# PKU-VCL-Geometry/GeoSplatting

Hardware: AMD Instinct MI355X
Metric: fwd+bwd views/sec at 2M Gaussians, 800x800 (higher is better)
Workload: dtype f32

## Files before the change

### geosplatting_amd/csrc/gs_cube.h

```cpp
#pragma once
#include "gs_common.h"

struct FaceMap { int a, b, c; float sx, sy; };
__device__ __forceinline__ FaceMap face_map(int s)
{
    const int axis = s >> 1;
    FaceMap m;
    m.a = axis == 0 ? 2 : 0;
    m.b = axis == 1 ? 2 : 1;
    m.c = axis;
    m.sx = (s == 0 || s == 5) ? -1.0f : 1.0f;
    m.sy = s == 2 ? 1.0f : -1.0f;
    return m;
}

__device__ __forceinline__ int select_face(const float* d)
{
    const float ax = fabsf(d[0]), ay = fabsf(d[1]), az = fabsf(d[2]);
    int f; float c;
    if (az > fmaxf(ax, ay)) { f = 4; c = d[2]; }
    else if (ay > ax)       { f = 2; c = d[1]; }
    else                    { f = 0; c = d[0]; }
    return f + (c < 0.0f ? 1 : 0);
}
// ... 12 lines not shown

__device__ __forceinline__ float comp3(const float* d, int i) { return i == 0 ? d[0] : (i == 1 ? d[1] : d[2]); }

__device__ __attribute__((noinline)) int resolve_texel_reproject(int s, int ix, int iy, int R)
{
    const float xn = 2.0f * (((float)ix + 0.5f) / (float)R) - 1.0f;
    const float yn = 2.0f * (((float)iy + 0.5f) / (float)R) - 1.0f;
    float p[3];
    face_point(s, xn, yn, p);
    const int s2 = select_face(p);
    const FaceMap m = face_map(s2);
    const float inv = 1.0f / fabsf(comp3(p, m.c));
    const float x2 = m.sx * comp3(p, m.a) * inv, y2 = m.sy * comp3(p, m.b) * inv;
    const float tx = (x2 + 1.0f) * 0.5f * (float)R - 0.5f, ty = (y2 + 1.0f) * 0.5f * (float)R - 0.5f;
    int jx = (int)floorf(tx + 0.5f), jy = (int)floorf(ty + 0.5f);
    jx = min(max(jx, 0), R - 1); jy = min(max(jy, 0), R - 1);
    return (s2 * R + jy) * R + jx;
}

#define GS_CUBE_EDGE_TABLE_MAX_R 4096
__device__ __forceinline__ int resolve_texel(int s, int ix, int iy, int R)
{
    const bool ox = (ix < 0 || ix >= R), oy = (iy < 0 || iy >= R);
    if (!ox && !oy) return (s * R + iy) * R + ix;
    if (ox && oy) return -1;
    const int e = ox ? (ix < 0 ? 0 : 1) : (iy < 0 ? 2 : 3);
    const int t = ox ? iy : ix;
    const unsigned w = s == 0 ? 0x97aa2ccu : s == 1 ? 0xc70a24du : s == 2 ? 0x2874c11u : s == 3 ? 0x7ad1839u : s == 4 ? 0x26ca049u : 0x766a0c8u;
    const unsigned c = (w >> (7 * e)) & 127u;
    const int s2 = (int)(c & 7u), kx = (int)((c >> 3) & 3u), ky = (int)((c >> 5) & 3u);
    const int jx = kx == 0 ? 0 : (kx == 1 ? R - 1 : (kx == 2 ? t : R - 1 - t));
    const int jy = ky == 0 ? 0 : (ky == 1 ? R - 1 : (ky == 2 ? t : R - 1 - t));
    return (s2 * R + jy) * R + jx;
}

struct CubeFp {
    bool valid;
    int idx[4];
    float w[4];
    float fx, fy;
    int face;
    float inv_c, xn, yn;
};

__device__ void cube_footprint(const float* d, int R, CubeFp& fp)
{
    const int s = select_face(d);
    const FaceMap m = face_map(s);
    const float ac = fabsf(comp3(d, m.c));
    fp.valid = (ac > 0.0f) && isfinite(ac);
    fp.face = s;
    if (!fp.valid) { fp.idx[0] = fp.idx[1] = fp.idx[2] = fp.idx[3] = 0; return; }
    const float inv = 1.0f / ac;
    const float xn = m.sx * comp3(d, m.a) * inv, yn = m.sy * comp3(d, m.b) * inv;
    fp.inv_c = inv; fp.xn = xn; fp.yn = yn;
    const float tx = (xn + 1.0f) * 0.5f * (float)R - 0.5f, ty = (yn + 1.0f) * 0.5f * (float)R - 0.5f;
    const int ix0 = (int)floorf(tx), iy0 = (int)floorf(ty);
    const float fx = tx - (float)ix0, fy = ty - (float)iy0;
    fp.fx = fx; fp.fy = fy;
    if (ix0 >= 0 && iy0 >= 0 && ix0 + 1 < R && iy0 + 1 < R) {
        const int b = (s * R + iy0) * R + ix0;
        fp.idx[0] = b; fp.idx[1] = b + 1; fp.idx[2] = b + R; fp.idx[3] = b + R + 1;
    } else {
        fp.idx[0] = resolve_texel(s, ix0, iy0, R);
        fp.idx[1] = resolve_texel(s, ix0 + 1, iy0, R);
        fp.idx[2] = resolve_texel(s, ix0, iy0 + 1, R);
        fp.idx[3] = resolve_texel(s, ix0 + 1, iy0 + 1, R);
    }
    float w[4] = { (1.0f - fx) * (1.0f - fy), fx * (1.0f - fy), (1.0f - fx) * fy, fx * fy };
    int miss = -1;
#pragma unroll
    for (int i = 0; i < 4; ++i) if (fp.idx[i] < 0) miss = i;
#pragma unroll
    for (int i = 0; i < 4; ++i) fp.w[i] = w[i];
    if (miss >= 0) {
        float wm = 0.0f;
#pragma unroll
        for (int i = 0; i < 4; ++i) if (i == miss) wm = w[i] / 3.0f;
#pragma unroll
        for (int i = 0; i < 4; ++i) fp.w[i] = (i == miss) ? 0.0f : w[i] + wm;
    }
}

template <bool WITH_GRAD>
__device__ void cube_fetch(const float* __restrict__ tex, int R, const float* d, float* out, float* dd, CubeFp& fp)
{
    cube_footprint(d, R, fp);
    const bool valid = fp.valid;
    bool ok[4]; int safe[4];
#pragma unroll
    for (int i = 0; i < 4; ++i) { ok[i] = valid && fp.idx[i] >= 0; safe[i] = ok[i] ? fp.idx[i] : 0; }
    float t[4][3];
#pragma unroll
    for (int i = 0; i < 4; ++i) {
        const float* p = tex + (size_t)safe[i] * 3;
        t[i][0] = p[0]; t[i][1] = p[1]; t[i][2] = p[2];
    }
    bool has_miss = false;
#pragma unroll
    for (int i = 0; i < 4; ++i) {
        if (!ok[i]) { t[i][0] = t[i][1] = t[i][2] = 0.0f; }
        has_miss = has_miss || (valid && fp.idx[i] < 0);
    }
    if (has_miss) {
#pragma unroll
        for (int c = 0; c < 3; ++c) {
            const float s = (t[0][c] + t[1][c] + t[2][c] + t[3][c]) / 3.0f;
#pragma unroll
            for (int i = 0; i < 4; ++i) if (fp.idx[i] < 0) t[i][c] = s;
        }
    }
    if (!valid) {
        out[0] = out[1] = out[2] = 0.0f;
        if (WITH_GRAD) { for (int i = 0; i < 9; ++i) dd[i] = 0.0f; }
        return;
    }
    const FaceMap m = face_map(fp.face);
    const float sgn_c = comp3(d, m.c) < 0.0f ? -1.0f : 1.0f;
#pragma unroll
    for (int c = 0; c < 3; ++c) {
        const float top = t[0][c] + fp.fx * (t[1][c] - t[0][c]);
        const float bot = t[2][c] + fp.fx * (t[3][c] - t[2][c]);
        out[c] = top + fp.fy * (bot - top);
        if (WITH_GRAD) {
            const float dtx = (t[1][c] - t[0][c]) + fp.fy * ((t[3][c] - t[2][c]) - (t[1][c] - t[0][c]));
            const float dty = bot - top;
            const float gx = dtx * 0.5f * (float)R, gy = dty * 0.5f * (float)R;
            float g[3] = { 0.0f, 0.0f, 0.0f };
            const float va = gx * m.sx * fp.inv_c, vb = gy * m.sy * fp.inv_c;
            const float vc = -(gx * fp.xn + gy * fp.yn) * fp.inv_c * sgn_c;
#pragma unroll
            for (int k = 0; k < 3; ++k) g[k] = (k == m.a ? va : 0.0f) + (k == m.b ? vb : 0.0f) + (k == m.c ? vc : 0.0f);
            dd[c * 3 + 0] = g[0]; dd[c * 3 + 1] = g[1]; dd[c * 3 + 2] = g[2];
        }
    }
}

template <bool XCD_LOCAL>
__device__ __forceinline__ void gs_add_scoped(float* p, float v)
{
    if (XCD_LOCAL) gs_atomic_add_xcd(p, v); else gs_atomic_add(p, v);
}

template <bool XCD_LOCAL>
__device__ __forceinline__ void wave_commit6_lds(float* stage, float* pa, float* pb, const float (&v)[6])
{
    const int lane = (int)(threadIdx.x & 63);
    unsigned long long* sp = reinterpret_cast<unsigned long long*>(stage);
    float* sv = stage + 256;
    __builtin_amdgcn_wave_barrier();
    sp[lane] = (unsigned long long)pa; sp[64 + lane] = (unsigned long long)pb;
#pragma unroll
    for (int c = 0; c < 6; ++c) sv[c * 64 + lane] = v[c];
    __builtin_amdgcn_fence(__ATOMIC_RELEASE, "wavefront");
    __builtin_amdgcn_wave_barrier();
    __builtin_amdgcn_fence(__ATOMIC_ACQUIRE, "wavefront");
#pragma unroll
    for (int k = 0; k < 6; ++k) {
        const int q = 64 * k + lane;
        const int src = q / 6, ch = q - 6 * src;
        const bool second = ch >= 3;
        float* base = (float*)sp[(second ? 64 : 0) + src];
        const float val = sv[ch * 64 + src];
        if (base != nullptr) gs_add_scoped<XCD_LOCAL>(base + (second ? ch - 3 : ch), val);
    }
}
// ... 86 lines not shown
```

### geosplatting_amd/csrc/gs_shade.hip

```cpp
#include "gs_common.h"
#include <stdlib.h>
#include <math.h>

#pragma clang fp contract(off)
#include "gs_shade_dev.h"

__global__ void __launch_bounds__(256)
shade_fwd_kernel(int N, const float* __restrict__ means, const float* __restrict__ normals,
                 const float* __restrict__ kd, const float* __restrict__ ks, const float* __restrict__ cam_pos,
                 float min_roughness, float max_metallic, int mode, EnvDev env, float* __restrict__ colors)
{
    const int n = blockIdx.x * blockDim.x + threadIdx.x;
    if (n >= N) return;
    const float mean[3] = { means[3 * (size_t)n], means[3 * (size_t)n + 1], means[3 * (size_t)n + 2] };
    const float nrm[3] = { normals[3 * (size_t)n], normals[3 * (size_t)n + 1], normals[3 * (size_t)n + 2] };
    const float kdn[3] = { kd[3 * (size_t)n], kd[3 * (size_t)n + 1], kd[3 * (size_t)n + 2] };
    const float2 ks2 = *reinterpret_cast<const float2*>(ks + 2 * (size_t)n);
    const float ksn[2] = { ks2.x, ks2.y };
    const float cp[3] = { cam_pos[0], cam_pos[1], cam_pos[2] };
    ShadeTmp t;
    float color[3];
    shade_one<false>(mean, nrm, kdn, ksn, cp, min_roughness, max_metallic, mode, env, color, t);
    colors[3 * (size_t)n] = color[0]; colors[3 * (size_t)n + 1] = color[1]; colors[3 * (size_t)n + 2] = color[2];
}

template <bool PRIV>
__global__ void __launch_bounds__(GS_SHADE_BWD_BLOCK)
shade_bwd_kernel(int N, const float* __restrict__ means, const float* __restrict__ normals,
                 const float* __restrict__ kd, const float* __restrict__ ks, const float* __restrict__ cam_pos,
                 float min_roughness, float max_metallic, int mode, EnvDev env, const float* __restrict__ v_colors,
                 float* __restrict__ v_means, float* __restrict__ v_normals, float* __restrict__ v_kd,
                 float* __restrict__ v_ks, EnvGradDev eg, int accumulate)
{
    extern __shared__ __attribute__((aligned(16))) float s_grad[];
    for (int i = threadIdx.x; i < eg.lds_floats; i += blockDim.x) s_grad[i] = 0.0f;
    __syncthreads();
    float* const priv = PRIV ? eg.priv + (long long)gs_xcc_id() * eg.priv_stride : nullptr;
    float* const stage = s_grad + eg.stage_off + (threadIdx.x >> 6) * 640;
    const float cp[3] = { cam_pos[0], cam_pos[1], cam_pos[2] };
    const int n_iter = (N + (int)(gridDim.x * blockDim.x) - 1) / (int)(gridDim.x * blockDim.x);
    for (int it = 0; it < n_iter; ++it) {
        const int n = it * (int)(gridDim.x * blockDim.x) + blockIdx.x * blockDim.x + threadIdx.x;
        bool scatter = false;
        ShadeTmp t;
        float v_ls[3] = { 0, 0, 0 }, v_ld[3] = { 0, 0, 0 };
        if (n < N) {
            const float mean[3] = { means[3 * (size_t)n], means[3 * (size_t)n + 1], means[3 * (size_t)n + 2] };
            const float normal[3] = { normals[3 * (size_t)n], normals[3 * (size_t)n + 1], normals[3 * (size_t)n + 2] };
            const float kdn[3] = { kd[3 * (size_t)n], kd[3 * (size_t)n + 1], kd[3 * (size_t)n + 2] };
            const float2 ks2 = *reinterpret_cast<const float2*>(ks + 2 * (size_t)n);
            const float ksn[2] = { ks2.x, ks2.y };
            const float g[3] = { v_colors[3 * (size_t)n], v_colors[3 * (size_t)n + 1], v_colors[3 * (size_t)n + 2] };
            if (g[0] == 0.0f && g[1] == 0.0f && g[2] == 0.0f) {
#pragma unroll
                for (int k = 0; k < 3; ++k) {
                    if (!accumulate) { v_means[3 * (size_t)n + k] = 0.0f; v_normals[3 * (size_t)n + k] = 0.0f; v_kd[3 * (size_t)n + k] = 0.0f; }
                }
                if (!accumulate) *reinterpret_cast<float2*>(v_ks + 2 * (size_t)n) = make_float2(0.0f, 0.0f);
            } else {
                float color[3], o_mean[3], v_n[3], o_kd[3], o_ks[2];
                shade_one<true>(mean, normal, kdn, ksn, cp, min_roughness, max_metallic, mode, env, color, t);
                shade_one_bwd(t, normal, kdn, g, mode, min_roughness, max_metallic, v_ls, v_ld, o_kd, v_n, o_ks, o_mean);
                scatter = true;
                if (accumulate) {
#pragma unroll
                    for (int k = 0; k < 3; ++k) {
                        v_means[3 * (size_t)n + k] += o_mean[k];
                        v_normals[3 * (size_t)n + k] += v_n[k];
                        v_kd[3 * (size_t)n + k] += o_kd[k];
                    }
                    float2 o = *reinterpret_cast<float2*>(v_ks + 2 * (size_t)n);
                    o.x += o_ks[0]; o.y += o_ks[1];
                    *reinterpret_cast<float2*>(v_ks + 2 * (size_t)n) = o;
                } else {
#pragma unroll
                    for (int k = 0; k < 3; ++k) {
                        v_means[3 * (size_t)n + k] = o_mean[k];
                        v_normals[3 * (size_t)n + k] = v_n[k];
                        v_kd[3 * (size_t)n + k] = o_kd[k];
                    }
                    *reinterpret_cast<float2*>(v_ks + 2 * (size_t)n) = make_float2(o_ks[0], o_ks[1]);
                }
            }
        }
        if (mode != GS_MODE_DIFFUSE) {
            const int l0 = scatter ? t.ls.l0 : 0, l1 = scatter ? t.ls.l1 : -1;
            const float w0 = (l1 < 0) ? 1.0f : 1.0f - t.ls.f;
            const bool lds0 = scatter && eg.lds_level[l0] >= 0;
            if (lds0) cube_scatter_lds(s_grad + eg.lds_level[l0], t.ls.fp0, v_ls, w0);
            cube_scatter_wave<PRIV>(scatter && !lds0 ? (PRIV ? priv + eg.priv_level[l0] : eg.levels[l0]) : nullptr, t.ls.fp0,
                                    v_ls, w0, scatter && !lds0, stage);
            const bool has1 = scatter && l1 >= 0;
            const bool lds1 = has1 && eg.lds_level[has1 ? l1 : 0] >= 0;
            if (lds1) cube_scatter_lds(s_grad + eg.lds_level[l1], t.ls.fp1, v_ls, t.ls.f);
            cube_scatter_wave<PRIV>(has1 && !lds1 ? (PRIV ? priv + eg.priv_level[has1 ? l1 : 0] : eg.levels[l1]) : nullptr,
                                    t.ls.fp1, v_ls, t.ls.f, has1 && !lds1, stage);
        } else {
            const bool ldsb = scatter && eg.lds_base >= 0;
            if (ldsb) cube_scatter_lds(s_grad + eg.lds_base, t.ld_fp, v_ld, 1.0f);
            cube_scatter_wave<PRIV>(scatter && !ldsb ? (PRIV ? priv + eg.priv_base : eg.base) : nullptr, t.ld_fp, v_ld, 1.0f,
                                    scatter && !ldsb, stage);
        }
    }
    __syncthreads();
    env_lds_flush(s_grad, eg, env);
// ... 131 lines not shown
        const float gx = g.x * tone_grad(mode, r * e), gy = g.y * tone_grad(mode, gch * e), gz = g.z * tone_grad(mode, b * e);
        v_render[3 * p] = gx * e; v_render[3 * p + 1] = gy * e; v_render[3 * p + 2] = gz * e;
        v_alphas[p] = mode == GS_TONE_NONE ? g.w * e : g.w;
        ve += gx * r + gy * gch + gz * b + (mode == GS_TONE_NONE ? g.w * a : 0.0f);
    }
    ve = gs_wave_sum(ve);
    __shared__ float s[4];
    if ((threadIdx.x & 63) == 0) s[threadIdx.x >> 6] = ve;
    __syncthreads();
    if (threadIdx.x == 0) gs_atomic_add(v_exposure, s[0] + s[1] + s[2] + s[3]);
}

extern "C" int gs_tonemap_fwd3(int64_t P, int mode, const float* render, const float* alphas, const float* exposure, float* out,
                               void* stream)
{
    GS_CHECK_ARG(P >= 0 && mode >= 0 && mode <= 2, "bad P or mode");
    if (P == 0) return GS_OK;
    const int blocks = (int)((P + 255) / 256 < 2048 ? (P + 255) / 256 : 2048);
    hipLaunchKernelGGL(tonemap_fwd3_kernel, dim3(blocks), dim3(256), 0, (hipStream_t)stream, P, mode, render, alphas, exposure, (float4*)out);
    GS_CHECK_LAUNCH();
    return GS_OK;
}

extern "C" int gs_tonemap_bwd3(int64_t P, int mode, const float* render, const float* alphas, const float* exposure,
                               const float* v_out, float* v_render, float* v_alphas, float* v_exposure, int accumulate, void* stream)
{
    GS_CHECK_ARG(P >= 0 && mode >= 0 && mode <= 2, "bad P or mode");
    hipStream_t s = (hipStream_t)stream;
    if (!accumulate) GS_CHECK_HIP(gs_zero_async(v_exposure, sizeof(float), s));
    if (P == 0) return GS_OK;
    const int blocks = (int)((P + 255) / 256 < 1024 ? (P + 255) / 256 : 1024);
    hipLaunchKernelGGL(tonemap_bwd3_kernel, dim3(blocks), dim3(256), 0, s, P, mode, render, alphas, exposure, (const float4*)v_out,
                       v_render, v_alphas, v_exposure);
    GS_CHECK_LAUNCH();
    return GS_OK;
}

extern "C" int gs_tonemap_fwd(int64_t P, int mode, const float* rgba, const float* exposure, float* out, void* stream)
{
    GS_CHECK_ARG(P >= 0 && mode >= 0 && mode <= 2, "bad P or mode");
    if (P == 0) return GS_OK;
    const int blocks = (int)((P + 255) / 256 < 2048 ? (P + 255) / 256 : 2048);
    hipLaunchKernelGGL(tonemap_fwd_kernel, dim3(blocks), dim3(256), 0, (hipStream_t)stream, P, mode,
                       (const float4*)rgba, exposure, (float4*)out);
    GS_CHECK_LAUNCH();
    return GS_OK;
}

extern "C" int gs_tonemap_bwd(int64_t P, int mode, const float* rgba, const float* exposure, const float* v_out,
                              float* v_rgba, float* v_exposure, int accumulate, void* stream)
{
    GS_CHECK_ARG(P >= 0 && mode >= 0 && mode <= 2, "bad P or mode");
    hipStream_t s = (hipStream_t)stream;
    if (!accumulate) GS_CHECK_HIP(gs_zero_async(v_exposure, sizeof(float), s));
    if (P == 0) return GS_OK;
    const int blocks = (int)((P + 255) / 256 < 1024 ? (P + 255) / 256 : 1024);
    hipLaunchKernelGGL(tonemap_bwd_kernel, dim3(blocks), dim3(256), 0, s, P, mode, (const float4*)rgba, exposure,
                       (const float4*)v_out, (float4*)v_rgba, v_exposure);
    GS_CHECK_LAUNCH();
    return GS_OK;
}

__global__ void __launch_bounds__(256) selftest_cube_edges_kernel(int R, unsigned long long* mismatches)
{
    const long long total = 24ll * R;
    unsigned long long bad = 0;
    for (long long i = (long long)blockIdx.x * blockDim.x + threadIdx.x; i < total; i += (long long)gridDim.x * blockDim.x) {
        const int t = (int)(i % R), e = (int)((i / R) & 3), s = (int)(i / (4ll * R));
        const int ix = e == 0 ? -1 : (e == 1 ? R : t), iy = e == 2 ? -1 : (e == 3 ? R : t);
        bad += resolve_texel(s, ix, iy, R) != resolve_texel_reproject(s, ix, iy, R);
    }
    if (bad) atomicAdd(mismatches, bad);
}

extern "C" int gs_selftest_cube_edges(int R, uint64_t* mismatches_dev, void* stream)
{
    GS_CHECK_ARG(mismatches_dev != nullptr && R >= 1 && R <= GS_CUBE_EDGE_TABLE_MAX_R, "bad size");
    hipStream_t s = (hipStream_t)stream;
    GS_CHECK_HIP(gs_zero_async(mismatches_dev, sizeof(uint64_t), s));
    hipLaunchKernelGGL(selftest_cube_edges_kernel, dim3(gs_cdiv(24 * R, 256)), dim3(256), 0, s, R, (unsigned long long*)mismatches_dev);
    GS_CHECK_LAUNCH();
    return GS_OK;
}
```

### geosplatting_amd/csrc/gs_shade_dev.h

```cpp
#pragma once
#include "gs_common.h"
#include <stdlib.h>
#include <math.h>
#include "gs_cube.h"

struct EnvDev {
    const float* lut; int lut_res;
    const float* base; int base_res;
    int L;
    const float* levels[GS_MAX_LEVELS];
    int res[GS_MAX_LEVELS];
    float min_r, max_r;
};
struct EnvGradDev {
    float* base;
    float* levels[GS_MAX_LEVELS];
    int lds_base;
    int lds_level[GS_MAX_LEVELS];
    int lds_floats;
    int stage_off;
    float* priv;
    long long priv_stride;
    long long priv_level[GS_MAX_LEVELS];
    long long priv_base;
// ... 53 lines not shown
    m.l0 = last ? L - 1 : lf;
    m.l1 = last ? -1 : lf + 1;
    m.f = last ? 0.0f : lam - (float)m.l0;
    m.clamped = last || (bias < 0.0f || bias > (float)(L - 1));
    return m;
}

struct MipSample {
    float out[3], dd[9], dmip[3];
    CubeFp fp0, fp1;
    float f;
    int l0, l1;
};

template <bool WITH_GRAD>
__device__ void cube_mip_fetch(const EnvDev& env, const float* d, float bias, MipSample& s)
{
    const int L = env.L;
    const float lam = fminf(fmaxf(bias, 0.0f), (float)(L - 1));
    const int lf = (int)floorf(lam);
    const bool last = lf >= L - 1;
    const int l0 = last ? L - 1 : lf;
    const int l1 = last ? L - 1 : lf + 1;
    const float f = last ? 0.0f : lam - (float)l0;
    float c0[3], c1[3], dd0[9], dd1[9];
    cube_fetch<WITH_GRAD>(env.levels[l0], env.res[l0], d, c0, dd0, s.fp0);
    cube_fetch<WITH_GRAD>(env.levels[l1], env.res[l1], d, c1, dd1, s.fp1);
    s.l0 = l0; s.l1 = last ? -1 : l1; s.f = f;
    const bool clamped = last || (bias < 0.0f || bias > (float)(L - 1));
#pragma unroll
    for (int c = 0; c < 3; ++c) {
        s.out[c] = c0[c] + f * (c1[c] - c0[c]);
        s.dmip[c] = clamped ? 0.0f : (c1[c] - c0[c]);
        if (WITH_GRAD) {
#pragma unroll
            for (int k = 0; k < 3; ++k) s.dd[c * 3 + k] = dd0[c * 3 + k] + f * (dd1[c * 3 + k] - dd0[c * 3 + k]);
        }
    }
}

struct ShadeTmp {
    float rough, metal, spec[3], diff[3];
    float wo[3], len; bool wo_const;
    float d, ndv, fg[2], dfg_du[2], dfg_dv[2];
    float refl[3], mip, dmip_dr;
    MipSample ls;
    float ld[3], ld_dd[9]; CubeFp ld_fp;
    float refl_c[3];
};

template <bool WITH_GRAD>
__device__ void shade_one(const float* mean, const float* normal, const float* kd, const float* ks, const float* cam_pos,
                          float min_roughness, float max_metallic, int mode, const EnvDev& env, float* color, ShadeTmp& t)
{
    t.rough = ks[0] * (1.0f - min_roughness) + min_roughness;
    t.metal = ks[1] * max_metallic;
#pragma unroll
    for (int c = 0; c < 3; ++c) {
        t.spec[c] = (1.0f - t.metal) * 0.04f + kd[c] * t.metal;
        t.diff[c] = kd[c] * (1.0f - t.metal);
    }
    const float v[3] = { cam_pos[0] - mean[0], cam_pos[1] - mean[1], cam_pos[2] - mean[2] };
    const float len = sqrtf(v[0] * v[0] + v[1] * v[1] + v[2] * v[2]);
    t.len = len;
    if (len < 1e-6f) { t.wo[0] = 0.0f; t.wo[1] = 0.0f; t.wo[2] = 1.0f; t.wo_const = true; }
    else { const float l = fmaxf(len, 1e-6f); t.wo[0] = v[0] / l; t.wo[1] = v[1] / l; t.wo[2] = v[2] / l; t.wo_const = false; }
    t.d = normal[0] * t.wo[0] + normal[1] * t.wo[1] + normal[2] * t.wo[2];
    t.ndv = fmaxf(t.d, 1e-6f);
    tex2d_linear_clamp2(env.lut, env.lut_res, env.lut_res, t.ndv, t.rough, t.fg, t.dfg_du, t.dfg_dv);
#pragma unroll
    for (int k = 0; k < 3; ++k) t.refl[k] = 2.0f * t.d * normal[k] - t.wo[k];
    t.mip = mip_from_roughness(t.rough, env.min_r, env.max_r, env.L, t.dmip_dr);
    if (mode != GS_MODE_DIFFUSE) cube_mip_fetch<WITH_GRAD>(env, t.refl, t.mip, t.ls);
    else { t.ls.out[0] = t.ls.out[1] = t.ls.out[2] = 0.0f; }
    if (mode == GS_MODE_DIFFUSE) cube_fetch<WITH_GRAD>(env.base, env.base_res, normal, t.ld, t.ld_dd, t.ld_fp);
    else { t.ld[0] = t.ld[1] = t.ld[2] = 0.0f; }
#pragma unroll
    for (int c = 0; c < 3; ++c) {
        t.refl_c[c] = t.spec[c] * t.fg[0] + t.fg[1];
        if (mode == GS_MODE_PBR)          color[c] = t.diff[c] + t.ls.out[c] * t.refl_c[c];
        else if (mode == GS_MODE_DIFFUSE) color[c] = t.ld[c] * t.diff[c];
        else                              color[c] = t.ls.out[c] * t.refl_c[c];
    }
}

__device__ __forceinline__ void shade_one_bwd(const ShadeTmp& t, const float* normal, const float* kd, const float* g, int mode,
                                              float min_roughness, float max_metallic, float* v_ls, float* v_ld, float* o_kd, float* v_n,
                                              float* v_ks, float* o_mean)
{
    float v_diff[3] = { 0, 0, 0 }, v_rf[3] = { 0, 0, 0 };
#pragma unroll
    for (int c = 0; c < 3; ++c) {
        if (mode == GS_MODE_PBR)          { v_diff[c] = g[c]; v_ls[c] = g[c] * t.refl_c[c]; v_rf[c] = g[c] * t.ls.out[c]; }
        else if (mode == GS_MODE_DIFFUSE) { v_ld[c] = g[c] * t.diff[c]; v_diff[c] = g[c] * t.ld[c]; }
        else                              { v_ls[c] = g[c] * t.refl_c[c]; v_rf[c] = g[c] * t.ls.out[c]; }
    }
    float v_A = 0.0f, v_B = 0.0f, v_metal = 0.0f;
#pragma unroll
    for (int c = 0; c < 3; ++c) {
        const float v_spec = v_rf[c] * t.fg[0];
        v_A += v_rf[c] * t.spec[c];
        v_B += v_rf[c];
        o_kd[c] = v_spec * t.metal + v_diff[c] * (1.0f - t.metal);
        v_metal += v_spec * (kd[c] - 0.04f) - v_diff[c] * kd[c];
    }
    const float v_ndv = v_A * t.dfg_du[0] + v_B * t.dfg_du[1];
    float v_rough = v_A * t.dfg_dv[0] + v_B * t.dfg_dv[1];
    float v_mip = 0.0f, v_refl[3] = { 0, 0, 0 };
    v_n[0] = v_n[1] = v_n[2] = 0.0f;
    if (mode != GS_MODE_DIFFUSE) {
#pragma unroll
        for (int c = 0; c < 3; ++c) {
            v_mip += v_ls[c] * t.ls.dmip[c];
#pragma unroll
            for (int k = 0; k < 3; ++k) v_refl[k] += v_ls[c] * t.ls.dd[c * 3 + k];
        }
    } else {
#pragma unroll
        for (int c = 0; c < 3; ++c)
#pragma unroll
            for (int k = 0; k < 3; ++k) v_n[k] += v_ld[c] * t.ld_dd[c * 3 + k];
    }
    v_rough += v_mip * t.dmip_dr;
    float v_d = 2.0f * (v_refl[0] * normal[0] + v_refl[1] * normal[1] + v_refl[2] * normal[2]);
    float v_wo[3];
#pragma unroll
    for (int k = 0; k < 3; ++k) { v_n[k] += 2.0f * t.d * v_refl[k]; v_wo[k] = -v_refl[k]; }
    if (t.d >= 1e-6f) v_d += v_ndv;
#pragma unroll
    for (int k = 0; k < 3; ++k) { v_n[k] += v_d * t.wo[k]; v_wo[k] += v_d * normal[k]; }
    o_mean[0] = o_mean[1] = o_mean[2] = 0.0f;
    if (!t.wo_const) {
        const float dot = t.wo[0] * v_wo[0] + t.wo[1] * v_wo[1] + t.wo[2] * v_wo[2];
        const float l = fmaxf(t.len, 1e-6f);
#pragma unroll
        for (int k = 0; k < 3; ++k) o_mean[k] = -((v_wo[k] - t.wo[k] * dot) / l);
    }
    v_ks[0] = v_rough * (1.0f - min_roughness); v_ks[1] = v_metal * max_metallic;
}

__device__ __forceinline__ void cube_fetch_vjp(const float* __restrict__ tex, int R, const float* d, const float* v, float* out,
                                               float& s, float* v_d, CubeFp& fp)
{
    cube_footprint(d, R, fp);
    const bool valid = fp.valid;
    bool ok[4]; int safe[4];
#pragma unroll
    for (int i = 0; i < 4; ++i) { ok[i] = valid && fp.idx[i] >= 0; safe[i] = ok[i] ? fp.idx[i] : 0; }
    float t[4][3];
#pragma unroll
    for (int i = 0; i < 4; ++i) {
        const float* p = tex + (size_t)safe[i] * 3;
        t[i][0] = p[0]; t[i][1] = p[1]; t[i][2] = p[2];
    }
    bool has_miss = false;
#pragma unroll
    for (int i = 0; i < 4; ++i) {
        if (!ok[i]) { t[i][0] = t[i][1] = t[i][2] = 0.0f; }
        has_miss = has_miss || (valid && fp.idx[i] < 0);
    }
    if (has_miss) {
#pragma unroll
        for (int c = 0; c < 3; ++c) {
            const float m = (t[0][c] + t[1][c] + t[2][c] + t[3][c]) / 3.0f;
#pragma unroll
            for (int i = 0; i < 4; ++i) if (fp.idx[i] < 0) t[i][c] = m;
// ... 261 lines not shown
```

### include/geosplat_hip.h

```cpp
#ifndef GEOSPLAT_HIP_H
#define GEOSPLAT_HIP_H

#include <stddef.h>
#include <stdint.h>

#ifdef __cplusplus
extern "C" {
#endif

#define GS_OK            0
#define GS_EINVAL       -1
#define GS_ENOSPC       -2
#define GS_ELAUNCH      -3

#define GS_MAX_LEVELS   16
#define GS_MAX_CHANNELS 32

#define GS_MODE_PBR      0
#define GS_MODE_DIFFUSE  1
#define GS_MODE_SPECULAR 2
#define GS_TONE_NONE     0
#define GS_TONE_NAIVE    1
#define GS_TONE_ACES     2

// ... 52 lines not shown
size_t gs_raster_ws_bytes(int64_t n_isects, int V, int W, int H, int tile_size);

int gs_raster_fwd(int W, int H, int tile_size, int D, int V, const float* means2d, const float* conics,
                  const float* opacities, const float* colors, const float* background,
                  int64_t n_isects, const int32_t* offsets, const int32_t* flatten_ids,
                  float* render, float* alphas, int32_t* last_ids, void* ws, size_t ws_bytes, void* stream);

int gs_raster_prepare(int W, int H, int tile_size, int D, int V, const float* means2d, const float* conics,
                      const float* opacities, const float* colors, int64_t n_isects, const int32_t* offsets,
                      const int32_t* flatten_ids, void* ws, size_t ws_bytes, void* stream);
int gs_raster_prepare_vis(int W, int H, int tile_size, int D, int V, const float* vis_records ,
                          int64_t n_isects, const int32_t* offsets, const int32_t* flatten_ids, void* ws, size_t ws_bytes,
                          void* stream);
int gs_raster_composite(int W, int H, int tile_size, int D, int V, const float* colors, const float* background,
                        int64_t n_isects, const int32_t* offsets, float* render, float* alphas, int32_t* last_ids,
                        const void* ws, size_t ws_bytes, void* stream);

int gs_raster_grad_stride(int D);

int gs_raster_bwd(int W, int H, int tile_size, int D, int V, const float* colors, const float* background,
                  int64_t n_isects, const int32_t* offsets, const float* alphas, const int32_t* last_ids,
                  const float* v_render, const float* v_alphas, float* v_packed, const void* ws, size_t ws_bytes,
                  void* stream);

int gs_raster_bwd_acc(int W, int H, int tile_size, int D, int V, const float* colors, const float* background,
                      int64_t n_isects, const int32_t* offsets, const float* alphas, const int32_t* last_ids,
                      const float* v_render, const float* v_alphas, float* v_packed, const void* ws, size_t ws_bytes,
                      void* stream);

int gs_isect_bin_cap(int V_cap, const float* means2d, const int32_t* radii, const float* depths, const int64_t* counts_dev,
                     int64_t n_isects_cap, int tile_size, int tile_w, int tile_h, int64_t* isect_ids_sorted,
                     int32_t* flatten_ids_sorted, void* ws, size_t ws_bytes, int64_t* status_dev, void* stream);
int gs_isect_offsets_cap(int64_t n_isects_cap, const int64_t* counts_dev, const int64_t* isect_ids_sorted, int n_tiles,
                         int32_t* offsets, void* stream);
int gs_isect_bin_tiles_cap(int V_cap, const float* means2d, const int32_t* radii, const float* depths, const int64_t* counts_dev,
                           int64_t n_isects_cap, int tile_size, int tile_w, int tile_h, int32_t* tile_ids_sorted,
                           int32_t* flatten_ids_sorted, void* ws, size_t ws_bytes, int64_t* status_dev, void* stream);
int gs_isect_offsets_tiles_cap(int64_t n_isects_cap, const int64_t* counts_dev, const int32_t* tile_ids_sorted, int n_tiles,
                               int32_t* offsets, void* stream);
int gs_raster_prepare_vis_cap(int W, int H, int tile_size, int D, int V_cap, const float* vis_records, int64_t n_isects_cap,
                              const int64_t* counts_dev, const int32_t* offsets, const int32_t* flatten_ids, void* ws,
                              size_t ws_bytes, void* stream);
int gs_raster_composite_cap(int W, int H, int tile_size, int D, int V_cap, const float* colors, const float* background,
                            int64_t n_isects_cap, const int64_t* counts_dev, const int32_t* offsets, float* render,
                            float* alphas, int32_t* last_ids, const void* ws, size_t ws_bytes, void* stream);
int gs_raster_bwd_cap(int W, int H, int tile_size, int D, int V_cap, const float* colors, const float* background,
                      int64_t n_isects_cap, const int64_t* counts_dev, const int32_t* offsets, const float* alphas,
                      const int32_t* last_ids, const float* v_render, const float* v_alphas, float* v_packed, const void* ws,
                      size_t ws_bytes, void* stream);
int gs_raster_bwd_acc_cap(int W, int H, int tile_size, int D, int V_cap, const float* colors, const float* background,
                          int64_t n_isects_cap, const int64_t* counts_dev, const int32_t* offsets, const float* alphas,
                          const int32_t* last_ids, const float* v_render, const float* v_alphas, float* v_packed, const void* ws,
                          size_t ws_bytes, void* stream);
int gs_raster_composite_tone(int W, int H, int tile_size, int V, const float* colors, int64_t n_isects,
                             const int64_t* counts_dev, const int32_t* offsets, float* render, float* alphas,
                             int32_t* last_ids, int tone_mode, const float* exposure , float* image,
                             const void* ws, size_t ws_bytes, void* stream);
int gs_raster_bwd_tone_acc(int W, int H, int tile_size, int V, const float* colors, int64_t n_isects,
                           const int64_t* counts_dev, const int32_t* offsets, const float* render, const float* alphas,
                           const int32_t* last_ids, int tone_mode, const float* exposure, const float* v_image,
                           float* v_packed, float* v_exposure, const void* ws, size_t ws_bytes, void* stream);
size_t gs_raster_log_ws_bytes(int64_t n_isects, int W, int H, int tile_size);
int gs_raster_composite_tone_log(int W, int H, int tile_size, int V, const float* colors, int64_t n_isects,
                                 const int64_t* counts_dev, const int32_t* offsets, float* render, float* alphas,
                                 int32_t* last_ids, int tone_mode, const float* exposure, float* image, const void* ws,
                                 size_t ws_bytes, void* log_ws, size_t log_bytes, void* stream);
int gs_raster_bwd_tone_log_acc(int W, int H, int tile_size, int V, const float* colors, int64_t n_isects,
                               const int64_t* counts_dev, const int32_t* offsets, const float* render, const float* alphas,
                               const int32_t* last_ids, int tone_mode, const float* exposure, const float* v_image,
                               float* v_packed, float* v_exposure, const void* ws, size_t ws_bytes, const void* log_ws,
                               size_t log_bytes, void* stream);
int gs_project_bwd_cap(int N, const int64_t* counts_dev, int D, const float* means, const float* quats, const float* scales,
                       const float* opacities, const float* viewmat, const float* K, int W, int H, float eps2d,
                       const int32_t* gaussian_ids, const float* conics, const float* compensations, const float* v_packed,
                       int rec_stride, const float* v_depths, float* v_means, float* v_quats, float* v_scales,
                       float* v_opacities, float* v_colors, int accumulate, void* stream);

int gs_selftest_rcp(uint32_t lo_bits, uint32_t hi_bits, uint64_t* mismatches_dev, void* stream);

int gs_selftest_exp(uint32_t lo_bits, uint32_t hi_bits, uint64_t* out_dev, void* stream);

int gs_selftest_cube_edges(int R, uint64_t* mismatches_dev, void* stream);

int gs_project_bwd(int N, int V, int D, const float* means, const float* quats, const float* scales,
                   const float* opacities, const float* viewmat, const float* K, int W, int H, float eps2d,
                   const int32_t* gaussian_ids, const float* conics, const float* compensations,
                   const float* v_packed, int rec_stride , const float* v_depths,
                   float* v_means, float* v_quats, float* v_scales, float* v_opacities, float* v_colors,
                   int accumulate, void* stream);

int gs_project_bwd_ex(int N, int V, int D, const float* means, const float* quats, const float* scales,
                      const float* opacities, const float* viewmat, const float* K, int W, int H, float eps2d,
                      const int32_t* gaussian_ids, const float* conics, const float* compensations,
                      const float* v_packed, int rec_stride, const float* v_depths, const float* sh_coeffs, int sh_K,
                      int sh_degree, int flags, float* v_means, float* v_quats, float* v_scales, float* v_opacities,
                      float* v_colors, float* g_sh_coeffs, int accumulate, void* stream);

typedef struct GsEnv {
    const float* lut;
    int          lut_res;
    const float* base;
    int          base_res;
    int          num_levels;
    const float* levels[GS_MAX_LEVELS];
    int          res[GS_MAX_LEVELS];
    float        min_roughness;
    float        max_roughness;
} GsEnv;

typedef struct GsEnvGrad {
    float* base;
    float* levels[GS_MAX_LEVELS];
} GsEnvGrad;

int gs_shade_fwd(int N, const float* means, const float* normals, const float* kd, const float* ks,
                 const float* cam_pos, float min_roughness, float max_metallic, int mode,
                 const GsEnv* env , float* colors, void* stream);

size_t gs_shade_bwd_ws_bytes(const GsEnv* env , int mode);
int gs_shade_bwd_plan_blocks(const GsEnv* env , int mode, int N, int* block_threads);

int gs_shade_bwd(int N, const float* means, const float* normals, const float* kd, const float* ks,
                 const float* cam_pos, float min_roughness, float max_metallic, int mode,
                 const GsEnv* env , const float* v_colors,
                 float* v_means, float* v_normals, float* v_kd, float* v_ks,
                 const GsEnvGrad* env_grad , int accumulate, void* ws, size_t ws_bytes, void* stream);

int gs_tonemap_fwd(int64_t P, int mode, const float* rgba, const float* exposure, float* out, void* stream);
int gs_tonemap_fwd3(int64_t P, int mode, const float* render, const float* alphas, const float* exposure, float* out, void* stream);
int gs_tonemap_bwd3(int64_t P, int mode, const float* render, const float* alphas, const float* exposure, const float* v_out,
                    float* v_render, float* v_alphas, float* v_exposure, int accumulate, void* stream);
int gs_tonemap_bwd(int64_t P, int mode, const float* rgba, const float* exposure, const float* v_out,
                   float* v_rgba, float* v_exposure, int accumulate, void* stream);

int gs_cubemap_mip_fwd(int R, int C, const float* in, float* out, void* stream);
int gs_cubemap_mip_chain_fwd(int R, int n_levels, const float* in, float* const* outs, void* stream);
int gs_cube_sample_linear(int64_t n, const float* tex, int R, const float* dirs, float scale, float* out,
                          void* stream);
int gs_cubemap_mip_bwd(int R, const float* v_out, float* v_in, int accumulate, void* stream);
int gs_diffuse_cubemap_fwd(int R, const float* cubemap, float* out, void* stream);
int gs_diffuse_cubemap_bwd(int R, const float* v_out, float* v_cubemap, int accumulate, void* stream);
int gs_specular_bounds(int R, float costheta_cutoff, float* bounds, void* stream);
size_t gs_specular_bounds_ws_bytes(int R);
int gs_specular_bounds_fast(int R, float costheta_cutoff, const float* dir_table, float* bounds, void* ws, size_t ws_bytes, void* stream);
int gs_cube_dir_table(int R, float* table, void* stream);
int gs_specular_cubemap_fwd(int R, const float* cubemap, const float* bounds, const float* dir_table,
                            float roughness, float costheta_cutoff, float* out, void* stream);
int gs_specular_cubemap_bwd(int R, const float* bounds, const float* dir_table, const float* v_out_rgb,
                            float roughness, float costheta_cutoff, float* v_cubemap, int accumulate, void* stream);

int gs_specular_tiles_count(int R, float roughness, float costheta_cutoff, int backward, int margin, int bw, int nb, const float* bounds,
                            const float* dir_table, const int32_t* tiles, int n_tiles, int32_t* row_counts, int32_t* extents,
                            uint64_t* pairs, void* stream);
int gs_specular_tiles_fill(int R, float roughness, float costheta_cutoff, int backward, int margin, int bw, int nb, const float* bounds,
                           const float* dir_table, const int32_t* tiles, int n_tiles, const int64_t* row_begin,
                           const int32_t* segments, int32_t* desc, float* weights, void* stream);
int gs_specular_tiles_check(int R, const float* bounds, const float* dir_table, uint64_t* out2, void* stream);
int gs_specular_tiles_apply(int R, int backward, int n_mirrors, int margin, int bw, int nb, const float* src, const float* scale,
                            const float* out_scale, const float* bounds, const int32_t* tiles, const int32_t* segments,
                            const int64_t* row_begin, const int32_t* row_counts, const int32_t* desc, const float* weights, float* dst,
                            int tile_begin, int tile_end, size_t lds_bytes, void* stream);

typedef struct GsTileLevel {
    int R, n_mirrors, margin, bw, nb, tile_begin, tile_end, reserved;
    const float* src; const float* scale; const float* out_scale; const float* bounds;
    const int32_t* tiles; const int32_t* segments; const int64_t* row_begin; const int32_t* row_counts; const int32_t* desc;
// ... 253 lines not shown
```

Measured before the change: 780.7.

## Restructure forward shading into branchless phases that issue all cube taps together

Rewrites the forward shade kernel as select, footprint, issue and blend phases separated by scheduling barriers, so the BRDF LUT loads and the texel loads for both mip levels are issued before any blending. Cube footprint and edge resolution become branchless selects using packed per-face edge words in place of table lookups and branches. The kernel is also specialised at compile time for diffuse versus specular modes. This aims to raise memory-level parallelism and cut divergence, at the cost of more live registers, and adds a selftest for bitwise agreement with the old footprint.

```diff
diff --git a/geosplatting_amd/csrc/gs_cube.h b/geosplatting_amd/csrc/gs_cube.h
--- a/geosplatting_amd/csrc/gs_cube.h
+++ b/geosplatting_amd/csrc/gs_cube.h
@@ -118,6 +118,104 @@
     }
 }
 
+template <class T> __device__ __forceinline__ T gs_sel(bool c, T a, T b) { return c ? a : b; }
+__device__ __forceinline__ int resolve_texel_sel(int s, unsigned w, int ix, int iy, int R)
+{
+    const bool ox = (ix < 0) | (ix >= R), oy = (iy < 0) | (iy >= R);
+    const int e = gs_sel(ox, gs_sel(ix < 0, 0, 1), gs_sel(iy < 0, 2, 3));
+    const int t = gs_sel(ox, iy, ix);
+    const unsigned c = (w >> (7 * e)) & 127u;
+    const int s2 = (int)(c & 7u), kx = (int)((c >> 3) & 3u), ky = (int)((c >> 5) & 3u);
+    const int rm = R - 1, rt = R - 1 - t;
+    const int jx = gs_sel(kx == 0, 0, gs_sel(kx == 1, rm, gs_sel(kx == 2, t, rt)));
+    const int jy = gs_sel(ky == 0, 0, gs_sel(ky == 1, rm, gs_sel(ky == 2, t, rt)));
+    const int across = (s2 * R + jy) * R + jx, inside = (s * R + iy) * R + ix;
+    return gs_sel(ox & oy, -1, gs_sel(ox | oy, across, inside));
+}
+
+__device__ __forceinline__ void cube_footprint_sel(const float* d, int R, CubeFp& fp)
+{
+    const float ax = fabsf(d[0]), ay = fabsf(d[1]), az = fabsf(d[2]);
+    const bool fz = az > fmaxf(ax, ay), fy_ = ay > ax;
+    const float dc = gs_sel(fz, d[2], gs_sel(fy_, d[1], d[0]));
+    const int s = gs_sel(fz, 4, gs_sel(fy_, 2, 0)) + gs_sel(dc < 0.0f, 1, 0);
+    const FaceMap m = face_map(s);
+    const float ac = fabsf(comp3(d, m.c));
+    const bool valid = (ac > 0.0f) & (bool)isfinite(ac);
+    fp.valid = valid;
+    fp.face = s;
+    const float inv = 1.0f / ac;
+    const float xn = m.sx * comp3(d, m.a) * inv, yn = m.sy * comp3(d, m.b) * inv;
+    fp.inv_c = gs_sel(valid, inv, 0.0f); fp.xn = gs_sel(valid, xn, 0.0f); fp.yn = gs_sel(valid, yn, 0.0f);
+    const float tx0 = (xn + 1.0f) * 0.5f * (float)R - 0.5f, ty0 = (yn + 1.0f) * 0.5f * (float)R - 0.5f;
+    const float tx = gs_sel(valid, tx0, 0.0f), ty = gs_sel(valid, ty0, 0.0f);
+    const int ix0 = (int)floorf(tx), iy0 = (int)floorf(ty);
+    const float fx = tx - (float)ix0, fy = ty - (float)iy0;
+    fp.fx = fx; fp.fy = fy;
+    unsigned ew = 0x766a0c8u;
+    ew = gs_sel(s == 4, 0x26ca049u, ew); ew = gs_sel(s == 3, 0x7ad1839u, ew); ew = gs_sel(s == 2, 0x2874c11u, ew);
+    ew = gs_sel(s == 1, 0xc70a24du, ew); ew = gs_sel(s == 0, 0x97aa2ccu, ew);
+    const int r0 = resolve_texel_sel(s, ew, ix0, iy0, R), r1 = resolve_texel_sel(s, ew, ix0 + 1, iy0, R);
+    const int r2 = resolve_texel_sel(s, ew, ix0, iy0 + 1, R), r3 = resolve_texel_sel(s, ew, ix0 + 1, iy0 + 1, R);
+    fp.idx[0] = gs_sel(valid, r0, 0); fp.idx[1] = gs_sel(valid, r1, 0); fp.idx[2] = gs_sel(valid, r2, 0); fp.idx[3] = gs_sel(valid, r3, 0);
+    const float w[4] = { (1.0f - fx) * (1.0f - fy), fx * (1.0f - fy), (1.0f - fx) * fy, fx * fy };
+    int miss = -1;
+#pragma unroll
+    for (int i = 0; i < 4; ++i) miss = gs_sel(fp.idx[i] < 0, i, miss);
+    const float wm = gs_sel(miss == 0, w[0], gs_sel(miss == 1, w[1], gs_sel(miss == 2, w[2], w[3]))) / 3.0f;
+#pragma unroll
+    for (int i = 0; i < 4; ++i) fp.w[i] = gs_sel(miss < 0, w[i], gs_sel(i == miss, 0.0f, w[i] + wm));
+}
+
+struct CubeTaps { float t[4][3]; };
+struct CubeBlendFp { float fx, fy; int state; };
+struct CubeTapIdx { int safe[4]; };
+__device__ __forceinline__ void cube_footprint_fwd(const float* d, int R, CubeTapIdx& a, CubeBlendFp& b)
+{
+    CubeFp fp;
+    cube_footprint_sel(d, R, fp);
+    int miss = -1;
+#pragma unroll
+    for (int i = 0; i < 4; ++i) {
+        a.safe[i] = gs_sel(fp.valid & (fp.idx[i] >= 0), fp.idx[i], 0);
+        miss = gs_sel(fp.idx[i] < 0, i, miss);
+    }
+    b.fx = fp.fx; b.fy = fp.fy; b.state = gs_sel(fp.valid, miss, -2);
+}
+__device__ __forceinline__ void cube_taps_issue(const float* __restrict__ tex, const CubeTapIdx& a, CubeTaps& q)
+{
+#pragma unroll
+    for (int i = 0; i < 4; ++i) {
+        const float* p = tex + (size_t)a.safe[i] * 3;
+        q.t[i][0] = p[0]; q.t[i][1] = p[1]; q.t[i][2] = p[2];
+    }
+}
+__device__ __forceinline__ void cube_taps_blend(const CubeBlendFp& b, const CubeTaps& q, float* out)
+{
+    const bool valid = b.state >= -1;
+    float t[4][3];
+#pragma unroll
+    for (int i = 0; i < 4; ++i) {
+        const bool ok = valid & (b.state != i);
+#pragma unroll
+        for (int c = 0; c < 3; ++c) t[i][c] = gs_sel(ok, q.t[i][c], 0.0f);
+    }
+    if (b.state >= 0) {
+#pragma unroll
+        for (int c = 0; c < 3; ++c) {
+            const float s = (t[0][c] + t[1][c] + t[2][c] + t[3][c]) / 3.0f;
+#pragma unroll
+            for (int i = 0; i < 4; ++i) t[i][c] = gs_sel(b.state == i, s, t[i][c]);
+        }
+    }
+#pragma unroll
+    for (int c = 0; c < 3; ++c) {
+        const float top = t[0][c] + b.fx * (t[1][c] - t[0][c]);
+        const float bot = t[2][c] + b.fx * (t[3][c] - t[2][c]);
+        out[c] = gs_sel(valid, top + b.fy * (bot - top), 0.0f);
+    }
+}
+
 template <bool WITH_GRAD>
 __device__ void cube_fetch(const float* __restrict__ tex, int R, const float* d, float* out, float* dd, CubeFp& fp)
 {
diff --git a/geosplatting_amd/csrc/gs_shade.hip b/geosplatting_amd/csrc/gs_shade.hip
--- a/geosplatting_amd/csrc/gs_shade.hip
+++ b/geosplatting_amd/csrc/gs_shade.hip
@@ -18,9 +18,9 @@
     const float2 ks2 = *reinterpret_cast<const float2*>(ks + 2 * (size_t)n);
     const float ksn[2] = { ks2.x, ks2.y };
     const float cp[3] = { cam_pos[0], cam_pos[1], cam_pos[2] };
-    ShadeTmp t;
     float color[3];
-    shade_one<false>(mean, nrm, kdn, ksn, cp, min_roughness, max_metallic, mode, env, color, t);
+    if (mode == GS_MODE_DIFFUSE) shade_fwd_phases<true>(mean, nrm, kdn, ksn, cp, min_roughness, max_metallic, mode, env, color);
+    else                         shade_fwd_phases<false>(mean, nrm, kdn, ksn, cp, min_roughness, max_metallic, mode, env, color);
     colors[3 * (size_t)n] = color[0]; colors[3 * (size_t)n + 1] = color[1]; colors[3 * (size_t)n + 2] = color[2];
 }
 
@@ -318,3 +318,39 @@
     GS_CHECK_LAUNCH();
     return GS_OK;
 }
+
+__global__ void __launch_bounds__(256) selftest_cube_footprint_kernel(long long n, const float* __restrict__ dirs, int R, unsigned long long* mismatches)
+{
+    unsigned long long bad = 0;
+    for (long long i = (long long)blockIdx.x * blockDim.x + threadIdx.x; i < n; i += (long long)gridDim.x * blockDim.x) {
+        const float d[3] = { dirs[3 * i], dirs[3 * i + 1], dirs[3 * i + 2] };
+        CubeFp a, b;
+        cube_footprint(d, R, a);
+        cube_footprint_sel(d, R, b);
+        bool same = a.valid == b.valid && a.face == b.face;
+#pragma unroll
+        for (int k = 0; k < 4; ++k) same = same && a.idx[k] == b.idx[k];
+        if (a.valid) {
+            same = same && __float_as_uint(a.fx) == __float_as_uint(b.fx) && __float_as_uint(a.fy) == __float_as_uint(b.fy)
+                        && __float_as_uint(a.inv_c) == __float_as_uint(b.inv_c) && __float_as_uint(a.xn) == __float_as_uint(b.xn)
+                        && __float_as_uint(a.yn) == __float_as_uint(b.yn);
+#pragma unroll
+            for (int k = 0; k < 4; ++k) same = same && __float_as_uint(a.w[k]) == __float_as_uint(b.w[k]);
+        }
+        bad += same ? 0ull : 1ull;
+    }
+    if (bad) atomicAdd(mismatches, bad);
+}
+
+extern "C" int gs_selftest_cube_footprint(int64_t n, const float* dirs, int R, uint64_t* mismatches_dev, void* stream)
+{
+    GS_CHECK_ARG(mismatches_dev != nullptr && n >= 0 && (n == 0 || dirs != nullptr) && R >= 1 && R <= GS_CUBE_EDGE_TABLE_MAX_R, "bad size");
+    hipStream_t s = (hipStream_t)stream;
+    GS_CHECK_HIP(gs_zero_async(mismatches_dev, sizeof(uint64_t), s));
+    if (n == 0) return GS_OK;
+    const long long blocks = (n + 255) / 256;
+    hipLaunchKernelGGL(selftest_cube_footprint_kernel, dim3((unsigned)(blocks < 4096 ? blocks : 4096)), dim3(256), 0, s, (long long)n, dirs, R,
+                       (unsigned long long*)mismatches_dev);
+    GS_CHECK_LAUNCH();
+    return GS_OK;
+}
diff --git a/geosplatting_amd/csrc/gs_shade_dev.h b/geosplatting_amd/csrc/gs_shade_dev.h
--- a/geosplatting_amd/csrc/gs_shade_dev.h
+++ b/geosplatting_amd/csrc/gs_shade_dev.h
@@ -159,6 +159,129 @@
         else if (mode == GS_MODE_DIFFUSE) color[c] = t.ld[c] * t.diff[c];
         else                              color[c] = t.ls.out[c] * t.refl_c[c];
     }
+}
+
+struct ShadeSel {
+    float diff[3], spec[3];
+    float dir[3];
+    float lut_fx, lut_fy; float2 lut[4];
+    const float* tex0; const float* tex1;
+    int R0, R1;
+    float f;
+};
+struct ShadeTaps { CubeTapIdx a0, a1; CubeBlendFp b0, b1; CubeTaps c0, c1; };
+
+template <bool DIFFUSE>
+__device__ __forceinline__ void shade_select(const float* mean, const float* normal, const float* kd, const float* ks, const float* cam_pos,
+                                             float min_roughness, float max_metallic, const EnvDev& env, ShadeSel& s)
+{
+    const float rough = ks[0] * (1.0f - min_roughness) + min_roughness;
+    const float metal = ks[1] * max_metallic;
+#pragma unroll
+    for (int c = 0; c < 3; ++c) {
+        s.spec[c] = (1.0f - metal) * 0.04f + kd[c] * metal;
+        s.diff[c] = kd[c] * (1.0f - metal);
+    }
+    if (DIFFUSE) {
+        s.tex0 = env.base; s.tex1 = nullptr; s.R0 = env.base_res; s.R1 = 0; s.f = 0.0f;
+        s.dir[0] = normal[0]; s.dir[1] = normal[1]; s.dir[2] = normal[2];
+        return;
+    }
+    const float v[3] = { cam_pos[0] - mean[0], cam_pos[1] - mean[1], cam_pos[2] - mean[2] };
+    const float len = sqrtf(v[0] * v[0] + v[1] * v[1] + v[2] * v[2]);
+    const float l = fmaxf(len, 1e-6f);
+    const bool at_cam = len < 1e-6f;
+    const float wo[3] = { gs_sel(at_cam, 0.0f, v[0] / l), gs_sel(at_cam, 0.0f, v[1] / l), gs_sel(at_cam, 1.0f, v[2] / l) };
+    const float d = normal[0] * wo[0] + normal[1] * wo[1] + normal[2] * wo[2];
+    const float ndv = fmaxf(d, 1e-6f);
+    {
+        const int W = env.lut_res, H = env.lut_res;
+        const float x0 = ndv * (float)W - 0.5f, y0 = rough * (float)H - 0.5f, xm = (float)(W - 1), ym = (float)(H - 1);
+        const float x = gs_sel(x0 < 0.0f, 0.0f, gs_sel(x0 > xm, xm, x0)), y = gs_sel(y0 < 0.0f, 0.0f, gs_sel(y0 > ym, ym, y0));
+        const int ix0 = (int)floorf(x), iy0 = (int)floorf(y);
+        s.lut_fx = x - (float)ix0; s.lut_fy = y - (float)iy0;
+        const int ix1 = min(ix0 + 1, W - 1), iy1 = min(iy0 + 1, H - 1);
+        s.lut[0] = *reinterpret_cast<const float2*>(env.lut + ((size_t)iy0 * W + ix0) * 2);
+        s.lut[1] = *reinterpret_cast<const float2*>(env.lut + ((size_t)iy0 * W + ix1) * 2);
+        s.lut[2] = *reinterpret_cast<const float2*>(env.lut + ((size_t)iy1 * W + ix0) * 2);
+        s.lut[3] = *reinterpret_cast<const float2*>(env.lut + ((size_t)iy1 * W + ix1) * 2);
+    }
+#pragma unroll
+    for (int k = 0; k < 3; ++k) s.dir[k] = 2.0f * d * normal[k] - wo[k];
+    const int L = env.L;
+    float mip;
+    {
+        const float ta = (rough - env.min_r) / (env.max_r - env.min_r), tb = (rough - env.max_r) / (1.0f - env.max_r);
+        const float ma = fminf(fmaxf(ta, 0.0f), 1.0f) * (float)(L - 2), mb = fminf(fmaxf(tb, 0.0f), 1.0f) + (float)(L - 2);
+        mip = gs_sel(rough < env.max_r, ma, mb);
+    }
+    const float lam = fminf(fmaxf(mip, 0.0f), (float)(L - 1));
+    const int lf = (int)floorf(lam);
+    const bool last = lf >= L - 1;
+    const int l0 = gs_sel(last, L - 1, lf);
+    const int l1 = gs_sel(last, L - 1, lf + 1);
+    s.f = gs_sel(last, 0.0f, lam - (float)l0);
+    s.tex0 = env.levels[l0]; s.tex1 = env.levels[l1];
+    s.R0 = env.res[l0]; s.R1 = env.res[l1];
+}
+
+template <bool DIFFUSE>
+__device__ __forceinline__ void shade_footprints(ShadeSel& s, ShadeTaps& q)
+{
+    if (!DIFFUSE) {
+        float fg[2];
+        const float a00[2] = { s.lut[0].x, s.lut[0].y }, a10[2] = { s.lut[1].x, s.lut[1].y };
+        const float a01[2] = { s.lut[2].x, s.lut[2].y }, a11[2] = { s.lut[3].x, s.lut[3].y };
+#pragma unroll
+        for (int c = 0; c < 2; ++c) {
+            const float top = a00[c] + s.lut_fx * (a10[c] - a00[c]);
+            const float bot = a01[c] + s.lut_fx * (a11[c] - a01[c]);
+            fg[c] = top + s.lut_fy * (bot - top);
+        }
+#pragma unroll
+        for (int c = 0; c < 3; ++c) s.spec[c] = s.spec[c] * fg[0] + fg[1];
+    }
+    cube_footprint_fwd(s.dir, s.R0, q.a0, q.b0);
+    if (!DIFFUSE) cube_footprint_fwd(s.dir, s.R1, q.a1, q.b1);
+}
+template <bool DIFFUSE>
+__device__ __forceinline__ void shade_issue(const ShadeSel& s, ShadeTaps& q)
+{
+    cube_taps_issue(s.tex0, q.a0, q.c0);
+    if (!DIFFUSE) cube_taps_issue(s.tex1, q.a1, q.c1);
+}
+
+template <bool DIFFUSE>
+__device__ __forceinline__ void shade_blend(const ShadeSel& s, const ShadeTaps& q, bool pbr, float* color)
+{
+    float c0[3];
+    cube_taps_blend(q.b0, q.c0, c0);
+    if (DIFFUSE) {
+#pragma unroll
+        for (int c = 0; c < 3; ++c) color[c] = c0[c] * s.diff[c];
+        return;
+    }
+    float c1[3];
+    cube_taps_blend(q.b1, q.c1, c1);
+#pragma unroll
+    for (int c = 0; c < 3; ++c) {
+        const float ls = c0[c] + s.f * (c1[c] - c0[c]);
+        color[c] = gs_sel(pbr, s.diff[c] + ls * s.spec[c], ls * s.spec[c]);
+    }
+}
+
+template <bool DIFFUSE>
+__device__ __forceinline__ void shade_fwd_phases(const float* mean, const float* normal, const float* kd, const float* ks, const float* cam_pos,
+                                                 float min_roughness, float max_metallic, int mode, const EnvDev& env, float* color)
+{
+    ShadeSel sel;
+    ShadeTaps taps;
+    shade_select<DIFFUSE>(mean, normal, kd, ks, cam_pos, min_roughness, max_metallic, env, sel);
+    __builtin_amdgcn_sched_barrier(0);
+    shade_footprints<DIFFUSE>(sel, taps);
+    shade_issue<DIFFUSE>(sel, taps);
+    __builtin_amdgcn_sched_barrier(0);
+    shade_blend<DIFFUSE>(sel, taps, mode == GS_MODE_PBR, color);
 }
 
 __device__ __forceinline__ void shade_one_bwd(const ShadeTmp& t, const float* normal, const float* kd, const float* g, int mode,
diff --git a/include/geosplat_hip.h b/include/geosplat_hip.h
--- a/include/geosplat_hip.h
+++ b/include/geosplat_hip.h
@@ -158,6 +158,8 @@
 
 int gs_selftest_cube_edges(int R, uint64_t* mismatches_dev, void* stream);
 
+int gs_selftest_cube_footprint(int64_t n, const float* dirs, int R, uint64_t* mismatches_dev, void* stream);
+
 int gs_project_bwd(int N, int V, int D, const float* means, const float* quats, const float* scales,
                    const float* opacities, const float* viewmat, const float* K, int W, int H, float eps2d,
                    const int32_t* gaussian_ids, const float* conics, const float* compensations,
```

Measured after the change: 780.1, median of 2. No clear change (-0.1%).
